# dacase/rnamotif

Hardware: AMD Instinct MI355X
Metric: Mbases scanned/sec (whole node) + hits/sec, trna.descr (higher is better)
Workload: dtype u8; 1 GPU; trna.descr (15 elements) over 100 x 1000000 base synthetic records per GPU (iid uniform acgt, numpy default_rng(20240601)), both strands; database resident in HBM (no upload in the step); bases_per_gpu=100000000, total_bases=100000000, candidates=5837, parallelism=1 GPU

## Files before the change

### rnamotif_amd/csrc/rm_efn2_core.h

```cpp
#pragma once
#include "rm_efn_core.h"

#define RME2_INF	RMA_EFN2_INFINITY
template< class Cand, int BIG = 0 >
struct rme2_ctx_t {
	static constexpr int	max_helix = BIG ? 52 : 16, stk = BIG ? 128 : 32;
	const rma_efn2data_t	*E;
	const Cand	*C;
	int	l_base;
	RMD_FN_MEMBER int	bc( int i ) const { return C->bc( i ); }
	RMD_FN_MEMBER int	bp( int i ) const { return C->bp( i ); }
};

RMD_FN int rme2_min( int a, int b ) { return a < b ? a : b; }

template< class X > RMD_FN int rme2_aupen( const X &x, int i, int j )
{
	return ( x.bc( i ) == RMA_BC_T || x.bc( j ) == RMA_BC_T ) ? x.E->auend : 0;
}
template< class X > RMD_FN int rme2_dangle( const X &x, int i, int j, int ip, int jp )
{
	return x.E->dangle[ x.bc( i ) ][ x.bc( j ) ][ x.bc( ip ) ][ jp ];
}
template< class X > RMD_FN int rme2_loginc( const X &x, int size )
// ... 101 lines not shown
	}
	if( closed )
		coax[ n ][ n ] = coax[ 0 ][ 0 ];
	const int	npair = closed ? n : n - 1;
	for( int h = 0; h < npair; h++ ){
		const int	d = hx[ h + 1 ][ 1 ] - hx[ h ][ 0 ];
		int	v = coax[ h ][ h ] + coax[ h + 1 ][ h + 1 ];
		if( d == 1 )
			v = rme2_min( v, RME2_T4( coax, hx[ h ][ 1 ], hx[ h ][ 0 ], hx[ h + 1 ][ 1 ], hx[ h + 1 ][ 0 ] ) );
		else if( d == 2 ){
			bool	g5, g3;
			if( closed ){
				g5 = h != 0 ? hx[ h ][ 1 ] - hx[ h - 1 ][ 0 ] > 1 : hx[ 0 ][ 1 ] - hx[ n - 1 ][ 0 ] > 1;
				g3 = h != n - 1 ? hx[ h + 2 ][ 1 ] - hx[ h + 1 ][ 0 ] > 1 : hx[ 1 ][ 1 ] - hx[ 0 ][ 0 ] > 1;
			}else{
				g5 = h != 0 ? hx[ h ][ 1 ] - hx[ h - 1 ][ 0 ] > 1 : hx[ 0 ][ 1 ] > 1;
				g3 = h != n - 2 ? hx[ h + 2 ][ 1 ] - hx[ h + 1 ][ 0 ] > 1 : hx[ n - 1 ][ 0 ] < l_base;
			}
			if( g5 ){
				const int	t = h != 0 ?
					RME2_T4( tstackcoax, hx[ h ][ 0 ], hx[ h ][ 1 ], hx[ h ][ 0 ] + 1, hx[ h ][ 1 ] - 1 ) :
					RME2_T4( tstackcoax, hx[ h ][ 1 ], hx[ h ][ 0 ], hx[ h ][ 0 ] + 1, hx[ h ][ 1 ] - 1 );
				v = rme2_min( v, t + RME2_T4( coaxstack, hx[ h ][ 0 ] + 1, hx[ h ][ 1 ] - 1, hx[ h + 1 ][ 1 ], hx[ h + 1 ][ 0 ] ) );
			}
			if( g3 )
				v = rme2_min( v, RME2_T4( tstackcoax, hx[ h ][ 0 ] + 1, hx[ h + 1 ][ 0 ] + 1, hx[ h + 1 ][ 1 ], hx[ h + 1 ][ 0 ] ) +
					RME2_T4( coaxstack, hx[ h ][ 0 ], hx[ h ][ 1 ], hx[ h ][ 0 ] + 1, hx[ h + 1 ][ 0 ] + 1 ) );
		}
		coax[ h ][ h + 1 ] = v;
	}
	for( int h = 2; h <= m && h < n; h++ )
		for( int a = 0; a + h <= m; a++ ){
			int	v = coax[ a ][ a ] + coax[ a + 1 ][ a + h ];
			for( int b = 1; b < h; b++ )
				v = rme2_min( v, coax[ a ][ a + b ] + coax[ a + b + 1 ][ a + h ] );
			coax[ a ][ a + h ] = v;
		}
	if( closed )
		return rme2_min( coax[ 0 ][ n - 1 ], coax[ 1 ][ n ] );
	return n >= 1 ? coax[ 0 ][ n - 1 ] : 0;
}

template< class X > RMD_FN int rme2_efn2( const X &x )
{
	const rma_efn2data_t	*e = x.E;
	const int	l_base = x.l_base;
	int	stk_i[ X::stk ], stk_j[ X::stk ], sp = 0;
	int	hx[ X::max_helix + 1 ][ 2 ];
	int	energy = 0;
	stk_i[ sp ] = 0;
	stk_j[ sp ] = l_base;
	sp++;
	while( sp > 0 ){
		sp--;
		int	i = stk_i[ sp ], j = stk_j[ sp ];
		if( i < 0 || j < 0 || i > l_base || j > l_base )
			return RME2_INF;
		if( x.bp( i ) == j ){
			if( i >= j )
				return RME2_INF;
			for( bool again = true; again; ){
				again = false;
				while( x.bp( i + 1 ) == j - 1 ){
					energy += RME2_T4( stack, i, j, i + 1, j - 1 ) + e->eparam[ 1 ];
					i++;
					j--;
				}
				int	n_helix = 0, ip = 0, jp = 0;
				for( int k = i + 1; k < j; ){
					const int	q = x.bp( k );
					if( q > k ){
						n_helix++;
						ip = k;
						k = q + 1;
						jp = q;
					}else if( q == -1 )
						k++;
					else
						return RME2_INF;
				}
				if( n_helix == 0 )
					energy += rme2_hploop( x, i, j );
				else if( n_helix == 1 ){
					energy += rme2_ibloop( x, i, j, ip, jp );
					i = ip;
					j = jp;
					again = true;
				}else{
					n_helix++;
					if( n_helix >= X::max_helix )
						return RME2_INF;
					hx[ 0 ][ 0 ] = i;
					hx[ 0 ][ 1 ] = j;
					int	n_upn = 0;
					for( int h = 1; h < n_helix; h++ ){
						int	p = hx[ h - 1 ][ 0 ] + 1;
						while( x.bp( p ) == -1 )
							p++;
						const int	q = x.bp( p );
						energy += rme2_aupen( x, p, q );
						hx[ h ][ 1 ] = p;
						hx[ h ][ 0 ] = q;
						if( sp >= X::stk )
							return RME2_INF;
						stk_i[ sp ] = p;
						stk_j[ sp ] = q;
						sp++;
						n_upn += p - hx[ h - 1 ][ 0 ] - 1;
					}
					hx[ n_helix ][ 0 ] = hx[ 0 ][ 0 ];
					hx[ n_helix ][ 1 ] = hx[ 0 ][ 1 ];
					n_upn += hx[ n_helix ][ 1 ] - hx[ n_helix - 1 ][ 0 ] - 1;
					energy += e->efn2a + n_helix * e->efn2c;
					energy += n_upn <= 6 ? n_upn * e->efn2b :
						6 * e->efn2b + e->mbl_log[ n_upn < RMA_EFN_LOGINC ? n_upn : RMA_EFN_LOGINC - 1 ];
					energy += rme2_branches( x, hx, n_helix, true );
				}
			}
			continue;
		}
		int	n_helix = 0;
		while( i < l_base ){
			const int	q = x.bp( i );
			if( q != -1 ){
				n_helix++;
				i = q;
			}
			i++;
		}
		if( n_helix >= X::max_helix )
			return RME2_INF;
		int	p = 1;
		for( int h = 0; h < n_helix; h++ ){
			while( p <= l_base && x.bp( p ) == 0 )
				p++;
			const int	q = p <= l_base ? x.bp( p ) : -1;
			if( q < 0 )
				return RME2_INF;
			energy += rme2_aupen( x, p, q );
			hx[ h ][ 1 ] = p;
			hx[ h ][ 0 ] = q;
			if( sp >= X::stk )
				return RME2_INF;
			stk_i[ sp ] = p;
			stk_j[ sp ] = q;
			sp++;
			p = q + 1;
		}
		energy += rme2_branches( x, hx, n_helix, false );
	}
	return energy;
}

template< class Seq, int BIG = 0 >
RMD_FN int rme2_site_energy( const rmd_program_t *P, const rma_efn2data_t *E, const Seq *sq, const int32_t *w, int k,
	int16_t *bpbuf = nullptr, uint8_t *bcbuf = nullptr, int cache = 0 )
{
	rme_cand_t<Seq>	c;
	c.P = P;
	c.w = w;
	c.sq = sq;
	if( !c.setup( rmd_efn_sites( P )[ k ] ) )
		return RME_INF;
	if( bpbuf != nullptr && c.len <= cache )
		c.fill_cache( bpbuf, bcbuf );
	rme2_ctx_t< rme_cand_t<Seq>, BIG >	x;
	x.E = E;
	x.C = &c;
	x.l_base = c.len - 1;
	return rme2_efn2( x );
}
```

### rnamotif_amd/csrc/rm_efn_core.h

```cpp
#pragma once
#include "rm_dev_program.h"

#ifndef RMD_FN
#define RMD_FN	static inline
#endif
#ifndef RMD_FN_MEMBER
#define RMD_FN_MEMBER	inline
#endif

enum {
	RME_INTER = 0,
	RME_BULGE = RME_INTER + 31,
	RME_HAIRPIN = RME_BULGE + 31,
	RME_DANGLE = RME_HAIRPIN + 31,
	RME_POPPEN = RME_DANGLE + 250,
	RME_EPARAM = RME_POPPEN + 5,
	RME_MISC = RME_EPARAM + 16,
	RME_TRIKEY = RME_MISC + 9,
	RME_TRIVAL = RME_TRIKEY + 50,
	RME_TLVAL = RME_TRIVAL + 50,
	RME_STACK = RME_TLVAL + 100,
	RME_TSTKH = RME_STACK + 625,
	RME_TSTKI = RME_TSTKH + 625,
	RME_SINT2 = RME_TSTKI + 625,
	RME_ASINT = RME_SINT2 + 900,
	RME_SINT4 = RME_ASINT + 4500,
	RME_N16 = RME_SINT4 + 22500
};
enum { RME_MAXPEN, RME_AUEND, RME_GUBONUS, RME_CSLOPE, RME_CINT, RME_C3, RME_GAIL, RME_NTRI, RME_NTL };

struct rme_tables_t {
	const int16_t	*t;
	const int32_t	*tlkey;
	const int32_t	*loginc;
};

template< class Cand, int BIG = 0 >
struct rme_ctx_t {
	static constexpr int	stk = BIG ? 128 : 48;
	const rme_tables_t	*T;
	const Cand	*C;
	int	l_base;
	RMD_FN_MEMBER int	bc( int i ) const { return C->bc( i ); }
	RMD_FN_MEMBER int	bp( int i ) const { return C->bp( i ); }
	RMD_FN_MEMBER int	tab( int off ) const { return T->t[ off ]; }
};

#define RME_INF	RMA_EFN_INFINITY

template< class X > RMD_FN int rme_dangle( const X &x, int i, int j, int ip, int jp )
{
	return x.tab( RME_DANGLE + ( ( x.bc( i ) * 5 + x.bc( j ) ) * 5 + x.bc( ip ) ) * 2 + jp );
}

template< class X > RMD_FN int rme_aupen( const X &x, int i, int j )
{
	int	bi = x.bc( i ), bj = x.bc( j );
	int	pen = ( bi == RMA_BC_A && bj == RMA_BC_T ) || ( bi == RMA_BC_G && bj == RMA_BC_T ) ||
		( bi == RMA_BC_T && ( bj == RMA_BC_A || bj == RMA_BC_G ) );
	return pen * x.tab( RME_MISC + RME_AUEND );
}

template< class X > RMD_FN int rme_tab4( const X &x, int base, int a, int b, int c, int d )
{
	return x.tab( base + ( ( a * 5 + b ) * 5 + c ) * 5 + d );
}

template< class X > RMD_FN int rme_loginc( const X &x, int size )
{
	return x.T->loginc[ size < RMA_EFN_LOGINC ? size : RMA_EFN_LOGINC - 1 ];
}

template< class X > RMD_FN int rme_stack( const X &x, int i, int j )
{
	if( i == x.l_base || j == x.l_base + 1 )
		return RME_INF;
	return rme_tab4( x, RME_STACK, x.bc( i ), x.bc( j ), x.bc( i + 1 ), x.bc( j - 1 ) ) + x.tab( RME_EPARAM + 0 );
}

RMD_FN int rme_wc( int i, int j ) { return i + j == 3; }
RMD_FN int rme_gu( int i, int j ) { return i == RMA_BC_G && j == RMA_BC_T; }

template< class X > RMD_FN int rme_ibloop( const X &x, int i, int j, int ip, int jp )
{
	if( ( i <= x.l_base && ip > x.l_base ) || ( jp <= x.l_base && j > x.l_base ) )
		return RME_INF;
	int	size1 = ip - i - 1, size2 = j - jp - 1, size = size1 + size2;
	int	m = size1 < size2 ? size1 : size2;
	int	min4 = m < 4 ? m : 4;
	int	si = x.bc( i ), sj = x.bc( j ), sip = x.bc( ip ), sjp = x.bc( jp );
	int	rval = 0;
	if( size1 == 0 || size2 == 0 ){
		if( size == 1 )
			return rme_tab4( x, RME_STACK, si, sj, sip, sjp ) + x.tab( RME_BULGE + size ) + x.tab( RME_EPARAM + 1 );
		rval = rme_aupen( x, i, j ) + rme_aupen( x, ip, jp );
		if( size > 30 )
			rval += x.tab( RME_BULGE + 30 ) + rme_loginc( x, size ) + x.tab( RME_EPARAM + 1 );
		else
			rval += x.tab( RME_BULGE + size ) + x.tab( RME_EPARAM + 1 );
		return rval;
	}
	int	lopsid = size1 > size2 ? size1 - size2 : size2 - size1;
	int	pen = lopsid * x.tab( RME_POPPEN + min4 );
	if( pen > x.tab( RME_MISC + RME_MAXPEN ) )
		pen = x.tab( RME_MISC + RME_MAXPEN );
	int	gail = ( size1 == 1 || size2 == 1 ) && x.tab( RME_MISC + RME_GAIL ) == 1;
	if( size > 30 ){
		if( gail )
			rval += rme_tab4( x, RME_TSTKI, si, sj, RMA_BC_A, RMA_BC_A ) + rme_tab4( x, RME_TSTKI, sjp, sip, RMA_BC_A, RMA_BC_A );
		else
			rval += rme_tab4( x, RME_TSTKI, si, sj, x.bc( i + 1 ), x.bc( j - 1 ) ) +
				rme_tab4( x, RME_TSTKI, sjp, sip, x.bc( jp + 1 ), x.bc( ip - 1 ) );
		rval += x.tab( RME_INTER + 30 ) + rme_loginc( x, size ) + x.tab( RME_EPARAM + 2 ) + pen;
	}else if( lopsid == 1 && size == 3 ){
		int	lf, rt;
		if( size1 < size2 ){
			if( rme_wc( si, sj ) ) lf = si;
			else if( rme_gu( si, sj ) ) lf = 4;
			else if( rme_gu( sj, si ) ) lf = 5;
			else return RME_INF;
			if( rme_wc( sip, sjp ) ) rt = sip;
			else if( rme_gu( sip, sjp ) ) rt = 4;
			else if( rme_gu( sjp, sip ) ) rt = 5;
			else return RME_INF;
			rval += x.tab( RME_EPARAM + 2 ) + x.tab( RME_ASINT + ( ( ( lf * 6 + rt ) * 5 + x.bc( i + 1 ) ) * 5 + x.bc( j - 1 ) ) * 5 + x.bc( jp + 1 ) );
		}else{
			if( rme_wc( sjp, sip ) ) lf = sjp;
			else if( rme_gu( sjp, sip ) ) lf = 4;
			else if( rme_gu( sip, sjp ) ) lf = 5;
			else return RME_INF;
			if( rme_wc( sj, si ) ) rt = sj;
			else if( rme_gu( sj, si ) ) rt = 4;
			else if( rme_gu( si, sj ) ) rt = 5;
			else return RME_INF;
			rval += x.tab( RME_EPARAM + 2 ) + x.tab( RME_ASINT + ( ( ( lf * 6 + rt ) * 5 + x.bc( jp + 1 ) ) * 5 + x.bc( ip - 1 ) ) * 5 + x.bc( i + 1 ) );
		}
	}else if( lopsid == 0 && size <= 4 ){
		int	lf, rt;
		if( rme_wc( si, sj ) ) lf = si;
		else if( rme_gu( si, sj ) || rme_gu( sj, si ) ) lf = si + 2;
		else return RME_INF;
		if( rme_wc( sip, sjp ) ) rt = sip;
		else if( rme_gu( sip, sjp ) || rme_gu( sjp, sip ) ) rt = sip + 2;
		else return RME_INF;
		if( size == 2 )
			rval += x.tab( RME_EPARAM + 2 ) + x.tab( RME_SINT2 + ( ( lf * 6 + rt ) * 5 + x.bc( i + 1 ) ) * 5 + x.bc( j - 1 ) );
		else if( size == 4 )
			rval += x.tab( RME_EPARAM + 2 ) + x.tab( RME_SINT4 + ( ( ( ( lf * 6 + rt ) * 5 + x.bc( i + 1 ) ) * 5 + x.bc( j - 1 ) ) * 5 + x.bc( ip - 1 ) ) * 5 + x.bc( jp + 1 ) );
	}else{
		if( gail )
			rval += rme_tab4( x, RME_TSTKI, si, sj, RMA_BC_A, RMA_BC_A ) + rme_tab4( x, RME_TSTKI, sjp, sip, RMA_BC_A, RMA_BC_A );
		else
			rval += rme_tab4( x, RME_TSTKI, si, sj, x.bc( i + 1 ), x.bc( j - 1 ) ) +
				rme_tab4( x, RME_TSTKI, sjp, sip, x.bc( jp + 1 ), x.bc( ip - 1 ) );
// ... 65 lines not shown
	int	sp = 0, e = 0;
	stk_i[ 0 ] = 0;
	stk_j[ 0 ] = x.l_base;
	stk_open[ 0 ] = 1;
	sp = 1;
	const int	fbp = x.tab( RME_EPARAM + 5 ), helixp = x.tab( RME_EPARAM + 8 );
	while( sp > 0 ){
		sp--;
		int	i = stk_i[ sp ], j = stk_j[ sp ];
		int	open = int( ( stk_open[ sp >> 6 ] >> ( sp & 63 ) ) & 1 );
		int	fb = open ? 0 : fbp;
		int	done = 0;
		const int	e_call = e;
		if( x.bp( i ) == -1 || x.bp( j ) == -1 ){
			while( x.bp( i ) == -1 && x.bp( i + 1 ) == -1 ){
				i++;
				e += fb;
				if( i >= j - 1 ){
					done = 1;
					break;
				}
			}
			if( done )
				continue;
			while( x.bp( j ) == -1 && x.bp( j - 1 ) == -1 ){
				j--;
				e += fb;
				if( i >= j - 1 ){
					done = 1;
					break;
				}
			}
			if( done )
				continue;
			if( x.bp( i ) == -1 && x.bp( i + 1 ) > i + 1 ){
				int	dg = rme_dangle( x, x.bp( i + 1 ), i + 1, i, 1 );
				e += ( dg < 0 ? dg : 0 ) + fb;
				i++;
			}
			if( x.bp( j ) == -1 && x.bp( j - 1 ) != -1 && x.bp( j - 1 ) < j - 1 ){
				int	dg = rme_dangle( x, j - 1, x.bp( j - 1 ), j, 0 );
				e += ( dg < 0 ? dg : 0 ) + fb;
				j--;
			}
		}
		if( x.bp( i ) != j ){
			int	k = x.bp( i ), kp = x.bp( j );
			if( k >= kp || sp + 2 > RME_STK ){
				e = e_call + RME_INF;
				continue;
			}
			int	cut;
			if( x.bp( k + 1 ) != -1 )
				cut = k;
			else if( x.bp( k + 2 ) == -1 )
				cut = k + 1;
			else if( rme_dangle( x, k, i, k + 1, 0 ) <= rme_dangle( x, x.bp( k + 2 ), k + 2, k + 1, 1 ) )
				cut = k + 1;
			else
				cut = k;
			stk_i[ sp ] = cut + 1;
			stk_j[ sp ] = j;
			stk_open[ sp >> 6 ] = ( stk_open[ sp >> 6 ] & ~( 1ull << ( sp & 63 ) ) ) | ( ( unsigned long long )open << ( sp & 63 ) );
			sp++;
			stk_i[ sp ] = i;
			stk_j[ sp ] = cut;
			stk_open[ sp >> 6 ] = ( stk_open[ sp >> 6 ] & ~( 1ull << ( sp & 63 ) ) ) | ( ( unsigned long long )open << ( sp & 63 ) );
			sp++;
			continue;
		}
		if( !open )
			e += helixp;
		e += rme_aupen( x, i, j );
		for( ; ; ){
			if( x.bp( i + 1 ) == j - 1 ){
				e += rme_stack( x, i, j );
				i++;
				j--;
				continue;
			}
			int	sum = 0, ip = 0, jp = 0, bad = 0;
			for( int k = i + 1; k < j; ){
				int	b = x.bp( k );
				if( b > k ){
					sum++;
					ip = k;
					k = b + 1;
					jp = k - 1;
					if( k > j ){
						bad = 1;
						break;
					}
				}else if( b == -1 )
					k++;
				else{
					bad = 1;
					break;
				}
			}
			if( bad ){
				e = e_call + RME_INF;
				break;
			}
			if( sum == 0 ){
				e += rme_hploop( x, i, j );
				break;
			}
			if( sum == 1 ){
				e += rme_ibloop( x, i, j, ip, jp );
				i = ip;
				j = jp;
				continue;
			}
			int	is = i + 1, js = j - 1;
			e += x.tab( RME_EPARAM + 4 ) + helixp + rme_aupen( x, i, j );
			if( x.bp( i + 1 ) == -1 && x.bp( i + 2 ) != -1 ){
				int	dg = rme_dangle( x, i, j, i + 1, 0 );
				if( dg <= rme_dangle( x, x.bp( i + 2 ), i + 2, i + 1, 1 ) ){
					is = i + 2;
					e += ( dg < 0 ? dg : 0 ) + fbp;
				}
			}
			if( x.bp( i + 1 ) == -1 && x.bp( i + 2 ) == -1 ){
				int	dg = rme_dangle( x, i, j, i + 1, 0 );
				is = i + 2;
				e += ( dg < 0 ? dg : 0 ) + fbp;
			}
			if( x.bp( j - 1 ) == -1 && x.bp( j - 2 ) != -1 ){
				int	dg = rme_dangle( x, i, j, j - 1, 1 );
				if( dg <= rme_dangle( x, j - 2, x.bp( j - 2 ), j - 1, 0 ) ){
					js = j - 2;
					e += ( dg < 0 ? dg : 0 ) + fbp;
				}
			}
			if( x.bp( j - 1 ) == -1 && x.bp( j - 2 ) == -1 ){
				int	dg = rme_dangle( x, i, j, j - 1, 1 );
				js = j - 2;
				e += ( dg < 0 ? dg : 0 ) + fbp;
			}
			if( sp + 1 > RME_STK ){
				e += RME_INF;
				break;
			}
			stk_i[ sp ] = is;
			stk_j[ sp ] = js;
			stk_open[ sp >> 6 ] &= ~( 1ull << ( sp & 63 ) );
			sp++;
			break;
		}
	}
	return e;
}

template< class Seq >
struct rme_cand_t {
	const rmd_program_t	*P;
	const int32_t	*w;
	const Seq	*sq;
	int	idx, idx2, pos, pos2;
	int	off5, start, len;
	int16_t	*cbp = nullptr;
	uint8_t	*cbc = nullptr;

	RMD_FN_MEMBER int	moff( int d ) const { return w[ RMA_HIT_HDR + 4 * d ]; }
	RMD_FN_MEMBER int	mlen( int d ) const { return w[ RMA_HIT_HDR + 4 * d + 1 ]; }

	RMD_FN_MEMBER int	setup( const rma_efn_site_t &es )
	{
		idx = es.idx;
		idx2 = es.idx2;
		pos = es.pos;
		pos2 = es.pos2 < 0 ? mlen( idx2 ) - 1 : es.pos2;
		off5 = moff( idx );
		start = off5 + pos;
		len = 0;
		for( int d = idx; d <= idx2; d++ ){
			int	t = P->elems[ d ].type;
			if( t != RMA_T_SS && t != RMA_T_H5 && t != RMA_T_H3 )
				return 0;
			len += mlen( d );
		}
		len -= pos;
		len -= mlen( idx2 ) - ( pos2 + 1 );
		if( len <= 0 )
			return 0;
		for( int d = idx; d <= idx2; d++ ){
			const rmd_elem_t	&st = P->elems[ d ];
			if( st.type == RMA_T_SS || ( st.type == RMA_T_H5 && d == idx2 ) || ( st.type == RMA_T_H3 && d == idx ) )
				continue;
			if( !st.proper )
				return 0;
			int	m = st.mates[ 0 ];
			int	p0 = d == idx ? pos : 0, p1 = d == idx2 ? pos2 + 1 : mlen( d );
			if( p0 >= p1 )
				continue;
			int	lo = ( mlen( m ) - ( p1 - 1 ) - 1 ) + moff( m ) - off5;
			int	hi = ( mlen( m ) - p0 - 1 ) + moff( m ) - off5;
			if( lo < 0 || hi >= len )
				return 0;
		}
		return 1;
	}
	RMD_FN_MEMBER void	fill_cache( int16_t *bpbuf, uint8_t *bcbuf )
	{
		for( int d = idx; d <= idx2; d++ ){
			const rmd_elem_t	&st = P->elems[ d ];
			const int	p0 = d == idx ? pos : 0, p1 = d == idx2 ? pos2 + 1 : mlen( d );
			const bool	ss = st.type == RMA_T_SS || ( st.type == RMA_T_H5 && d == idx2 ) || ( st.type == RMA_T_H3 && d == idx );
			const int	m = st.mates[ 0 ];
			const int	ps = P->efn_usestdbp ? P->efn_stdbp : st.pairset;
			for( int pq = p0; pq < p1; pq++ ){
				const int	p = moff( d ) + pq, i = p - start;
				const int	b = sq->code( p );
				bcbuf[ i ] = uint8_t( b );
				int	partner = -1;
				if( !ss ){
					const int	q1 = mlen( m ) - pq - 1;
					const int	b1 = sq->code( q1 + moff( m ) );
					if( ( rmd_pairsets( P )[ ps ].mat2 >> ( b * 5 + b1 ) ) & 1 )
						partner = q1 + moff( m ) - off5;
				}
				bpbuf[ i ] = int16_t( partner );
			}
		}
		cbp = bpbuf;
		cbc = bcbuf;
	}
	RMD_FN_MEMBER int	bc( int i ) const
	{
		if( i < 0 || i >= len )
			return RMA_BC_N;
		if( cbc != nullptr )
			return cbc[ i ];
		return sq->code( start + i );
	}
	RMD_FN_MEMBER int	bp( int i ) const
	{
		if( i < 0 || i >= len )
			return -1;
		if( cbp != nullptr )
			return cbp[ i ];
		int	p = start + i;
		for( int d = idx; d <= idx2; d++ ){
			int	o = moff( d ), l = mlen( d );
			if( p < o || p >= o + l )
				continue;
			const rmd_elem_t	&st = P->elems[ d ];
			if( st.type == RMA_T_SS || ( st.type == RMA_T_H5 && d == idx2 ) || ( st.type == RMA_T_H3 && d == idx ) )
				return -1;
			int	pq = p - o;
			int	m = st.mates[ 0 ];
			int	q1 = mlen( m ) - pq - 1;
			int	ps = P->efn_usestdbp ? P->efn_stdbp : st.pairset;
			int	b = sq->code( p ), b1 = sq->code( q1 + moff( m ) );
			return ( ( rmd_pairsets( P )[ ps ].mat2 >> ( b * 5 + b1 ) ) & 1 ) ? q1 + moff( m ) - off5 : -1;
		}
		return -1;
	}
};

template< class Seq, int BIG = 0 >
RMD_FN int rme_site_energy( const rmd_program_t *P, const rme_tables_t *T, const Seq *sq, const int32_t *w, int k,
	int16_t *bpbuf = nullptr, uint8_t *bcbuf = nullptr, int cache = 0 )
{
	rme_cand_t<Seq>	c;
	c.P = P;
	c.w = w;
	c.sq = sq;
	if( !c.setup( rmd_efn_sites( P )[ k ] ) )
		return RME_INF;
	if( bpbuf != nullptr && c.len <= cache )
		c.fill_cache( bpbuf, bcbuf );
	rme_ctx_t< rme_cand_t<Seq>, BIG >	x;
	x.T = T;
	x.C = &c;
	x.l_base = c.len - 1;
	return rme_efn( x );
}
```

### rnamotif_amd/csrc/rm_scan_kernel.h

```cpp
#pragma once
#include <hip/hip_runtime.h>
#include <cstdint>

#define RMD_HD		__host__ __device__ inline
#define RMD_FN		static __device__ inline
#define RMD_COLD	static __device__ inline
#define RMD_FN_MEMBER	__device__ inline
#include "rm_scan_core.h"
#include "rm_efn_core.h"
#include "rm_efn2_core.h"
#include "rm_kernels.h"

__device__ inline int db_code( const DbView &db, int64_t base )
{
	uint32_t	am = db.amask[ base >> 5 ];
	if( ( am >> ( base & 31 ) ) & 1 )
		return RMA_BC_N;
	return ( db.codes[ base >> 4 ] >> ( 2 * ( base & 15 ) ) ) & 3;
}

__device__ inline int db_strand_code( const DbView &db, int64_t off, int slen, int comp, int p )
{
	int	c = db_code( db, off + ( comp ? slen - 1 - p : p ) );
	return ( comp && c < 4 ) ? 3 - c : c;
// ... 1948 lines not shown
								int	whole;
								k = pool_item_begin<BLOCK>( P, db, pool + RMK_POOL_WORDS * size_t( i ), col, NIB_MAX, lr, st, nsq, sink.seq, sink.comp, whole );
							}else
								dry = true;
						}
						if( ( dbg & RMK_DBG_CYCLES ) && lane_id == 0 )
							atomicAdd( rmk_ctr<RMK_C_POP_CYCLES>( hb ), __builtin_amdgcn_s_memtime() - t_p0 );
						continue;
					}
					if( busy == 0 )
						break;
					const unsigned long long	t_s0 = ( dbg & RMK_DBG_CYCLES ) ? __builtin_amdgcn_s_memtime() : 0;
					if( ( dbg & RMK_DBG_CYCLES ) && lane_id == 0 ){
						atomicAdd( rmk_ctr<RMK_C_STEPS>( hb ), 1ull );
						atomicAdd( rmk_ctr<RMK_C_STEP_LANES>( hb ), ( unsigned long long )__popcll( busy ) );
					}
					int	k_in_ = 0;
					if( dbg & RMK_DBG_CYCLES ){
						k_in_ = k;
						for( int o = 32; o > 0; o >>= 1 )
							k_in_ = rmd_imax( k_in_, __shfl_xor( k_in_, o ) );
					}
					if( k >= 0 )
						k = rmd_lean_step<LdsRecs<BLOCK>, DevSink, rmd_nibseq_t<BLOCK>, rmd_no_accel_t, true>( P, lr, st, nsq, k, &lane, sink, none );
					const unsigned long long	t_e0 = ( dbg & RMK_DBG_CYCLES ) ? __builtin_amdgcn_s_memtime() : 0;
					const int	n_em_ = ( dbg & RMK_DBG_CYCLES ) ? __popcll( __ballot( k >= 0 && st.pending ) ) : 0;
					wave_emit_pending<BLOCK>( P, lr, st, k, [ & ]( int l ){
						return rmd_nibseq_t<BLOCK>{ nsq.w + ( l - lane_id ), __shfl( nsq.flip, l ), __shfl( nsq.bias, l ) }; },
						sink.seq, sink.comp, hb, lane_id );
					if( ( dbg & RMK_DBG_CYCLES ) && lane_id == 0 && n_em_ ){
						atomicAdd( rmk_ctr<RMK_C_EMIT_CYCLES>( hb ), __builtin_amdgcn_s_memtime() - t_e0 );
						atomicAdd( rmk_ctr<RMK_C_EMITTED>( hb ), ( unsigned long long )n_em_ );
					}
					if( ( dbg & RMK_DBG_CYCLES ) && lane_id == 0 ){
						const unsigned long long	dt_ = __builtin_amdgcn_s_memtime() - t_s0;
						atomicAdd( rmk_ctr<RMK_C_STEP_CYCLES>( hb ), dt_ );
						atomicMax( rmk_ctr<RMK_C_STEP_LONGEST>( hb ), dt_ );
						atomicAdd( rmk_ctr<RMK_C_STEP_LOG2>( hb ) + ( 63 - __clzll( dt_ | 1ull ) ), 1ull );
						atomicAdd( rmk_ctr<RMK_C_LEVEL_CYCLES>( hb ) + rmd_imin( rmd_imax( k_in_, 0 ), 15 ), dt_ );
						atomicAdd( rmk_ctr<RMK_C_LEVEL_STEPS>( hb ) + rmd_imin( rmd_imax( k_in_, 0 ), 15 ), 1ull );
						t_wave += dt_;
						atomicMax( rmk_ctr<RMK_C_WAVE_MOST>( hb ), t_wave );
					}
				}
				__syncthreads();
				if( tid == 0 ){
					s_pool_n = 0;
					s_pool_head = 0;
				}
			}
			if( last ){
				PHASE( 4 );
				if( ( dbg & RMK_DBG_TIMELINE ) && tid == 0 && had_tiles ){
					atomicMax( rmk_ctr<RMK_C_TL_DONE_MAX>( hb ), ( unsigned long long )wall_clock64() );
					atomicAdd( rmk_ctr<RMK_C_TL_DONE_SUM>( hb ), ( unsigned long long )wall_clock64() );
				}
				break;
			}
			}
		}else if constexpr( LEAN ){

			rmd_lean_t	st;
			TailAccel	accel{ P, pb, tile, pb_words, p_lo, vec_words * 64, tail_from_rows ? 0 : -1 };
			for( ; ; ){
				unsigned long long	t_b0 = ( dbg & RMK_DBG_CYCLES ) ? __builtin_amdgcn_s_memtime() : 0;
				for( unsigned long long want; ( want = __ballot( k < 0 && !dry ) ) != 0; ){
					if( ( dbg & RMK_DBG_CYCLES ) && lane_id == 0 ){
						atomicAdd( rmk_ctr<RMK_C_POP_ROUNDS>( hb ), 1ull );
						atomicAdd( rmk_ctr<RMK_C_POP_LANES>( hb ), ( unsigned long long )__popcll( want ) );
					}
					int	base = 0;
					if( lane_id == __ffsll( want ) - 1 )
						base = atomicAdd( &s_qhead, __popcll( want ) );
					base = __shfl( base, __ffsll( want ) - 1 );
					if( k < 0 && !dry ){
						const int	i = base + __popcll( want & lt_mask );
						if( i < nq ){
							const unsigned	item = i < qcap ? queue[ i ] :
								__hip_atomic_load( spill + ( i - qcap ), __ATOMIC_RELAXED, __HIP_MEMORY_SCOPE_AGENT );
							const int	r = int( item & 0xffffu );
							if constexpr( G > 1 ){
								const int	sl = int( item >> 26 );
								const int	*c = s_ctx[ sl ];
								slen = c[ 2 ];
								z0 = c[ 3 ];
								p_lo = c[ 4 ];
								tile = tile0 + size_t( sl ) * slot_bytes;
								pb = pb0 + ( size_t( sl ) * n_vec + 1 ) * pb_words;
								sq = rmd_seq_t{ tile, p_lo };
								sink.seq = c[ 0 ];
								sink.comp = c[ 1 ];
								accel.pb = pb;
								accel.tile = tile;
								accel.p_lo = p_lo;
								accel.vec_bits = c[ 5 ] * 64;
							}
							const int	szero = z0 + int( ( item >> 16 ) & ( G > 1 ? 0x3ffu : 0xffffu ) );
							bool	drop = false;
							if( accel.usable_for >= 0 && r != 0xffff ){
								int	hi, lo;
								rmd_level0_range( P, szero, slen, &hi, &lo );
								const int	span = hi - r - szero + 1;
								drop = true;
								for( int hl = e0.minlen; hl <= e0.maxlen && drop; hl++ ){
									const int	ilen = span - 2 * hl;
									if( ilen < e0.minilen )
										break;
									bool	ok;
									if( ilen <= e0.maxilen && ( !accel.tail( e0, szero, hl, span - 1 - hl, &ok ) || ok ) )
										drop = false;
								}
							}
							if( !drop )
								k = rmd_lean_begin( P, lr, st, szero, slen,
									r == 0xffff ? 0 : r, r == 0xffff ? RMD_ALL_RANKS : 1 );
						}else
							dry = true;
					}
				}
				const unsigned long long	busy = __ballot( k >= 0 );
				unsigned long long	t_b1 = 0;
				if( dbg & RMK_DBG_CYCLES ){
					t_b1 = __builtin_amdgcn_s_memtime();
					if( lane_id == 0 ){
						atomicAdd( rmk_ctr<RMK_C_POP_CYCLES>( hb ), t_b1 - t_b0 );
						atomicAdd( rmk_ctr<RMK_C_STEPS>( hb ), 1ull );
						atomicAdd( rmk_ctr<RMK_C_STEP_LANES>( hb ), ( unsigned long long )__popcll( busy ) );
					}
				}
				if( busy == 0 )
					break;
				if( k >= 0 )
					k = rmd_lean_step<LdsRecs<BLOCK>, DevSink, rmd_seq_t, TailAccel, true>( P, lr, st, sq, k, &lane, sink, accel );
				wave_emit_pending<BLOCK>( P, lr, st, k, [ & ]( int l ){
					return rmd_seq_t{ tile0 + __shfl( int( sq.sq - tile0 ), l ), __shfl( sq.sq0, l ) }; },
					sink.seq, sink.comp, hb, lane_id );
				if( ( dbg & RMK_DBG_CYCLES ) && lane_id == 0 )
					atomicAdd( rmk_ctr<RMK_C_STEP_CYCLES>( hb ), __builtin_amdgcn_s_memtime() - t_b1 );
			}
		}else{
			GenTile	gt{ P, lean_lo, g_before, g_deep, queue, spill, qcap, nq, &s_qhead, &s_dqn, &s_dqhead,
				pb, tile, pb_words, p_lo, vec_words, slen, z0, split_s, dbg,
				ConcatCtx{ db.base_off, db.slen, CONCAT ? db.concat_bases : 0ll, seq, ent_n } };
			general_pass_b<BLOCK, KINDS, CONCAT>( gt, sink );
		}
		PHASE( 4 );
		__syncthreads();
		PHASE( 5 );
	}
#undef PHASE
}

struct DevSeq {
	DbView	db;
	int64_t	off;
	int	slen, comp;
	__device__ inline int code( int p ) const { return db_strand_code( db, off, slen, comp, p ); }
};

#define RME_N16_PAD	( ( RME_N16 + 7 ) / 8 * 8 )
#define EFN_CACHE	96
#define EFN_LIGHT_LDS	( 64 * ( ( EFN_CACHE + 2 ) * 2 + EFN_CACHE + 4 ) )
template< int BLOCK, int BIG, bool STAGE >
__device__ __forceinline__ void efn_body( const rmd_program_t *gP, const DbView &db, int32_t *hits, long long n_hits,
	const int16_t *g16, const int32_t *tlkey, const int32_t *loginc, const rma_efn2data_t *e2 )
{
	__shared__ __align__( 16 ) int16_t	t16_s[ STAGE ? RME_N16_PAD : 8 ];
	const int16_t	*t16 = g16;
	if constexpr( STAGE ){
		if( g16 != nullptr )
			for( int i = threadIdx.x; i < RME_N16_PAD / 8; i += BLOCK )
				reinterpret_cast<uint4 *>( t16_s )[ i ] = reinterpret_cast<const uint4 *>( g16 )[ i ];
		__syncthreads();
		t16 = t16_s;
	}
	__shared__ int16_t	s_bp[ STAGE ? BLOCK : 1 ][ EFN_CACHE + 1 ];
	__shared__ uint8_t	s_bc[ STAGE ? BLOCK : 1 ][ EFN_CACHE + 4 ];
	rme_tables_t	T{ t16, tlkey, loginc };
	int16_t	*bpbuf = s_bp[ STAGE ? threadIdx.x : 0 ];
	uint8_t	*bcbuf = s_bc[ STAGE ? threadIdx.x : 0 ];
	if constexpr( !STAGE ){
		extern __shared__ __align__( 16 ) unsigned char	efn_dyn[];
		bpbuf = reinterpret_cast<int16_t *>( efn_dyn ) + threadIdx.x * ( EFN_CACHE + 2 );
		bcbuf = efn_dyn + BLOCK * ( EFN_CACHE + 2 ) * sizeof( int16_t ) + threadIdx.x * ( EFN_CACHE + 4 );
	}
	const int	efn_off = RMA_HIT_HDR + 4 * gP->n_elems + 4;
	for( long long h = ( long long )blockIdx.x * BLOCK + threadIdx.x; h < n_hits; h += ( long long )gridDim.x * BLOCK ){
		int32_t	*w = hits + h * gP->hit_stride;
		DevSeq	sq{ db, db.base_off[ w[ 0 ] ], db.slen[ w[ 0 ] ], w[ 1 ] };
		for( int k = 0; k < gP->n_efn; k++ ){
			if( rmd_efn_sites( gP )[ k ].kind == RMA_EFN_KIND_EFN2 )
				w[ efn_off + k ] = e2 != nullptr ? rme2_site_energy<DevSeq, BIG>( gP, e2, &sq, w, k, bpbuf, bcbuf, EFN_CACHE ) : RME2_INF;
			else if( g16 != nullptr )
				w[ efn_off + k ] = rme_site_energy<DevSeq, BIG>( gP, &T, &sq, w, k, bpbuf, bcbuf, EFN_CACHE );
		}
	}
}

template< int BLOCK, int BIG = 0 >
__global__ void __launch_bounds__( BLOCK )
rma_efn_kernel( const rmd_program_t *gP, DbView db, int32_t *hits, long long n_hits,
	const int16_t *g16, const int32_t *tlkey, const int32_t *loginc, const rma_efn2data_t *e2 )
{
	efn_body<BLOCK, BIG, true>( gP, db, hits, n_hits, g16, tlkey, loginc, e2 );
}

template< int BIG = 0 >
__global__ void __launch_bounds__( 64, 4 )
rma_efn_light_kernel( const rmd_program_t *gP, DbView db, int32_t *hits, long long n_hits,
	const int16_t *g16, const int32_t *tlkey, const int32_t *loginc, const rma_efn2data_t *e2 )
{
	__builtin_amdgcn_s_setprio( 3 );
	efn_body<64, BIG, false>( gP, db, hits, n_hits, g16, tlkey, loginc, e2 );
}

#define RMK_DEFINE_LAUNCHER( name_, LEAN_, G_, KINDS_, POOL_, ... ) \
hipError_t name_( int grid, size_t lds, hipStream_t s, const rmk_search_args &a ) \
{ \
	constexpr int	BLOCK_ = ( LEAN_ ) ? SEARCH_BLOCK : GENERAL_BLOCK; \
	auto	kernel = &rma_search_kernel<BLOCK_, LEAN_, G_, KINDS_, POOL_ __VA_OPT__(,) __VA_ARGS__>; \
	hipError_t	e = hipFuncSetAttribute( reinterpret_cast<const void *>( kernel ), hipFuncAttributeMaxDynamicSharedMemorySize, int( lds ) ); \
	if( e != hipSuccess ) \
		return e; \
	 \
	{ \
		static thread_local size_t	for_lds = ~size_t( 0 ); \
		static thread_local int	resident = 0, for_dev = -1; \
		int	dev = 0; \
		( void )hipGetDevice( &dev ); \
		if( for_lds != lds || for_dev != dev ){ \
			int	per_cu = 0, cus = 0; \
			resident = 0; \
			if( hipOccupancyMaxActiveBlocksPerMultiprocessor( &per_cu, kernel, BLOCK_, lds ) == hipSuccess && \
				hipDeviceGetAttribute( &cus, hipDeviceAttributeMultiprocessorCount, dev ) == hipSuccess ) \
				resident = per_cu * cus; \
			for_lds = lds; \
			for_dev = dev; \
		} \
		if( resident > 0 && grid > resident ) \
			grid = resident; \
	} \
	hipLaunchKernelGGL( kernel, dim3( grid ), dim3( BLOCK_ ), lds, s, \
		a.d_prog, a.prog_bytes, a.qcap, a.db, a.hb, a.tile_bytes, a.dbg ); \
	return hipGetLastError(); \
}

#define RMK_DEFINE_DRAIN_LAUNCHER( name_ ) \
hipError_t name_( int grid, size_t lds, hipStream_t s, const rmk_search_args &a ) \
{ \
	auto	kernel = &rma_drain_kernel<DRAIN_BLOCK>; \
	hipError_t	e = hipFuncSetAttribute( reinterpret_cast<const void *>( kernel ), hipFuncAttributeMaxDynamicSharedMemorySize, int( lds ) ); \
	if( e != hipSuccess ) \
		return e; \
	hipLaunchKernelGGL( kernel, dim3( grid ), dim3( DRAIN_BLOCK ), lds, s, a.d_prog, a.prog_bytes, a.db, a.hb, a.tile_bytes, a.dbg ); \
	return hipGetLastError(); \
}
```

Baseline: 165,900 Mbases/s.

## Decode EFN candidate base windows in bulk and stage element facts in LDS

The EFN cache fill now decodes a candidate's whole base window from a few packed code and ambiguity-mask words at once, instead of one strided global read per base. Partner bases are looked up in that local window. Per-element type, mate and pair-matrix facts are precomputed once per block into shared memory, so each candidate no longer walks the program struct and pairset table. Pointers are also marked restrict. The trade-offs are more register use for the unrolled word arrays and a block-wide sync at kernel start.

```diff
diff --git a/profiles/efn_window.py b/profiles/efn_window.py
--- /dev/null
+++ b/profiles/efn_window.py
@@ -0,0 +1,53 @@
+import json
+import os
+import statistics
+import sys
+import time
+
+ROOT = os.path.dirname(os.path.dirname(os.path.abspath(__file__)))
+sys.path.insert(0, ROOT)
+import rnamotif_amd as R
+
+tag, out = sys.argv[1], sys.argv[2]
+os.environ.setdefault("EFNDATA", R.EFNDATA_DIR)
+d = R.Descriptor(["-descr", os.path.join(ROOT, "tests", "golden", "descr", "trna.descr")])
+seqs = R.synthetic_records(100)
+scs = [R.Scanner(d), R.Scanner(d)]
+db = scs[0].database(seqs)
+for s in scs:
+    s.attach(db)
+
+
+def turns(n):
+    pend = None
+    for i in range(n):
+        s = scs[i & 1]
+        s.scan_begin(db)
+        if pend is not None:
+            pend.scan_end(copy=False)
+        pend = s
+    return pend.scan_end(copy=False).shape[0]
+
+
+row = {"lib": tag}
+for light in (1, 0):
+    scs[0].set_option("efn_light", light)
+    for rep in range(3):
+        scs[0].scan_device(db)
+    ks = []
+    for rep in range(12):
+        scs[0].scan_device(db)
+        ks.append(round(scs[0].last_kernel_ms()[2], 4))
+    row["efn_light_ms" if light else "efn_staged_ms"] = {"median": statistics.median(ks), "min": min(ks), "max": max(ks), "all": ks}
+scs[0].set_option("efn_light", -1)
+turns(20)
+ms = []
+for rep in range(5):
+    t0 = time.perf_counter()
+    cand = turns(200)
+    ms.append(round((time.perf_counter() - t0) / 200 * 1e3, 4))
+row["ms_per_step_in_turns"] = ms
+row["candidates"] = cand
+print(json.dumps(row), flush=True)
+with open(out, "a") as f:
+    f.write(json.dumps(row) + "\n")
diff --git a/rnamotif_amd/csrc/rm_efn2_core.h b/rnamotif_amd/csrc/rm_efn2_core.h
--- a/rnamotif_amd/csrc/rm_efn2_core.h
+++ b/rnamotif_amd/csrc/rm_efn2_core.h
@@ -277,19 +277,20 @@
 	return energy;
 }
 
-template< class Seq, int BIG = 0 >
+template< class Seq, int BIG = 0, bool FACTS = false >
 RMD_FN int rme2_site_energy( const rmd_program_t *P, const rma_efn2data_t *E, const Seq *sq, const int32_t *w, int k,
-	int16_t *bpbuf = nullptr, uint8_t *bcbuf = nullptr, int cache = 0 )
-{
-	rme_cand_t<Seq>	c;
+	int16_t *bpbuf = nullptr, uint8_t *bcbuf = nullptr, int cache = 0, const rme_el_t *el = nullptr )
+{
+	rme_cand_t<Seq, FACTS>	c;
 	c.P = P;
 	c.w = w;
 	c.sq = sq;
+	c.F = el;
 	if( !c.setup( rmd_efn_sites( P )[ k ] ) )
 		return RME_INF;
 	if( bpbuf != nullptr && c.len <= cache )
 		c.fill_cache( bpbuf, bcbuf );
-	rme2_ctx_t< rme_cand_t<Seq>, BIG >	x;
+	rme2_ctx_t< rme_cand_t<Seq, FACTS>, BIG >	x;
 	x.E = E;
 	x.C = &c;
 	x.l_base = c.len - 1;
diff --git a/rnamotif_amd/csrc/rm_efn_core.h b/rnamotif_amd/csrc/rm_efn_core.h
--- a/rnamotif_amd/csrc/rm_efn_core.h
+++ b/rnamotif_amd/csrc/rm_efn_core.h
@@ -1,5 +1,8 @@
 #pragma once
+#include <type_traits>
+#include <utility>
 #include "rm_dev_program.h"
+#include "rm_seq_window.h"
 
 #ifndef RMD_FN
 #define RMD_FN	static inline
@@ -371,11 +374,39 @@
 	return e;
 }
 
-template< class Seq >
+template< class Seq, class = void > struct rme_has_window : std::false_type {};
+template< class Seq > struct rme_has_window< Seq,
+	std::void_t< decltype( std::declval<const Seq &>().window( 0, 0, static_cast<uint8_t *>( nullptr ) ) ) > > : std::true_type {};
+
+struct rme_el_t {
+	uint32_t	mat2;
+	int8_t	type, proper, mate, pad;
+};
+RMD_FN rme_el_t rme_el_of( const rmd_program_t *P, int d )
+{
+	const rmd_elem_t	&st = P->elems[ d ];
+	rme_el_t	e{ 0, st.type, st.proper, st.mates[ 0 ], 0 };
+	if( st.type == RMA_T_H5 || st.type == RMA_T_H3 ){
+		const int	ps = P->efn_usestdbp ? P->efn_stdbp : st.pairset;
+		if( ps >= 0 )
+			e.mat2 = rmd_pairsets( P )[ ps ].mat2;
+	}
+	return e;
+}
+
+template< class Seq, bool FACTS = false >
 struct rme_cand_t {
 	const rmd_program_t	*P;
 	const int32_t	*w;
 	const Seq	*sq;
+	const rme_el_t	*F = nullptr;
+	RMD_FN_MEMBER rme_el_t	el( int d ) const
+	{
+		if constexpr( FACTS )
+			return F[ d ];
+		else
+			return rme_el_of( P, d );
+	}
 	int	idx, idx2, pos, pos2;
 	int	off5, start, len;
 	int16_t	*cbp = nullptr;
@@ -394,7 +425,7 @@
 		start = off5 + pos;
 		len = 0;
 		for( int d = idx; d <= idx2; d++ ){
-			int	t = P->elems[ d ].type;
+			int	t = el( d ).type;
 			if( t != RMA_T_SS && t != RMA_T_H5 && t != RMA_T_H3 )
 				return 0;
 			len += mlen( d );
@@ -404,12 +435,12 @@
 		if( len <= 0 )
 			return 0;
 		for( int d = idx; d <= idx2; d++ ){
-			const rmd_elem_t	&st = P->elems[ d ];
+			const rme_el_t	st = el( d );
 			if( st.type == RMA_T_SS || ( st.type == RMA_T_H5 && d == idx2 ) || ( st.type == RMA_T_H3 && d == idx ) )
 				continue;
 			if( !st.proper )
 				return 0;
-			int	m = st.mates[ 0 ];
+			int	m = st.mate;
 			int	p0 = d == idx ? pos : 0, p1 = d == idx2 ? pos2 + 1 : mlen( d );
 			if( p0 >= p1 )
 				continue;
@@ -422,24 +453,29 @@
 	}
 	RMD_FN_MEMBER void	fill_cache( int16_t *bpbuf, uint8_t *bcbuf )
 	{
+		if constexpr( rme_has_window<Seq>::value )
+			sq->window( start, len, bcbuf );
+		else
+			for( int i = 0; i < len; i++ )
+				bcbuf[ i ] = uint8_t( sq->code( start + i ) );
 		for( int d = idx; d <= idx2; d++ ){
-			const rmd_elem_t	&st = P->elems[ d ];
+			const rme_el_t	st = el( d );
+			const int	od = moff( d ) - start;
 			const int	p0 = d == idx ? pos : 0, p1 = d == idx2 ? pos2 + 1 : mlen( d );
 			const bool	ss = st.type == RMA_T_SS || ( st.type == RMA_T_H5 && d == idx2 ) || ( st.type == RMA_T_H3 && d == idx );
-			const int	m = st.mates[ 0 ];
-			const int	ps = P->efn_usestdbp ? P->efn_stdbp : st.pairset;
+			if( ss ){
+				for( int pq = p0; pq < p1; pq++ )
+					bpbuf[ od + pq ] = -1;
+				continue;
+			}
+			const int	m = st.mate;
+			const uint32_t	mat2 = st.mat2;
+			const int	qm = mlen( m ) - 1 + moff( m );
 			for( int pq = p0; pq < p1; pq++ ){
-				const int	p = moff( d ) + pq, i = p - start;
-				const int	b = sq->code( p );
-				bcbuf[ i ] = uint8_t( b );
-				int	partner = -1;
-				if( !ss ){
-					const int	q1 = mlen( m ) - pq - 1;
-					const int	b1 = sq->code( q1 + moff( m ) );
-					if( ( rmd_pairsets( P )[ ps ].mat2 >> ( b * 5 + b1 ) ) & 1 )
-						partner = q1 + moff( m ) - off5;
-				}
-				bpbuf[ i ] = int16_t( partner );
+				const int	b = bcbuf[ od + pq ];
+				const int	j = qm - pq - start;
+				const int	b1 = j >= 0 && j < len ? bcbuf[ j ] : sq->code( qm - pq );
+				bpbuf[ od + pq ] = int16_t( ( ( mat2 >> ( b * 5 + b1 ) ) & 1 ) ? qm - pq - off5 : -1 );
 			}
 		}
 		cbp = bpbuf;
@@ -464,33 +500,33 @@
 			int	o = moff( d ), l = mlen( d );
 			if( p < o || p >= o + l )
 				continue;
-			const rmd_elem_t	&st = P->elems[ d ];
+			const rme_el_t	st = el( d );
 			if( st.type == RMA_T_SS || ( st.type == RMA_T_H5 && d == idx2 ) || ( st.type == RMA_T_H3 && d == idx ) )
 				return -1;
 			int	pq = p - o;
-			int	m = st.mates[ 0 ];
+			int	m = st.mate;
 			int	q1 = mlen( m ) - pq - 1;
-			int	ps = P->efn_usestdbp ? P->efn_stdbp : st.pairset;
 			int	b = sq->code( p ), b1 = sq->code( q1 + moff( m ) );
-			return ( ( rmd_pairsets( P )[ ps ].mat2 >> ( b * 5 + b1 ) ) & 1 ) ? q1 + moff( m ) - off5 : -1;
+			return ( ( st.mat2 >> ( b * 5 + b1 ) ) & 1 ) ? q1 + moff( m ) - off5 : -1;
 		}
 		return -1;
 	}
 };
 
-template< class Seq, int BIG = 0 >
+template< class Seq, int BIG = 0, bool FACTS = false >
 RMD_FN int rme_site_energy( const rmd_program_t *P, const rme_tables_t *T, const Seq *sq, const int32_t *w, int k,
-	int16_t *bpbuf = nullptr, uint8_t *bcbuf = nullptr, int cache = 0 )
-{
-	rme_cand_t<Seq>	c;
+	int16_t *bpbuf = nullptr, uint8_t *bcbuf = nullptr, int cache = 0, const rme_el_t *el = nullptr )
+{
+	rme_cand_t<Seq, FACTS>	c;
 	c.P = P;
 	c.w = w;
 	c.sq = sq;
+	c.F = el;
 	if( !c.setup( rmd_efn_sites( P )[ k ] ) )
 		return RME_INF;
 	if( bpbuf != nullptr && c.len <= cache )
 		c.fill_cache( bpbuf, bcbuf );
-	rme_ctx_t< rme_cand_t<Seq>, BIG >	x;
+	rme_ctx_t< rme_cand_t<Seq, FACTS>, BIG >	x;
 	x.T = T;
 	x.C = &c;
 	x.l_base = c.len - 1;
diff --git a/rnamotif_amd/csrc/rm_scan_kernel.h b/rnamotif_amd/csrc/rm_scan_kernel.h
--- a/rnamotif_amd/csrc/rm_scan_kernel.h
+++ b/rnamotif_amd/csrc/rm_scan_kernel.h
@@ -2124,18 +2124,27 @@
 }
 
 struct DevSeq {
-	DbView	db;
+	const uint32_t	*codes, *amask;
 	int64_t	off;
 	int	slen, comp;
-	__device__ inline int code( int p ) const { return db_strand_code( db, off, slen, comp, p ); }
+	__device__ inline int code( int p ) const
+	{
+		const int64_t	base = off + ( comp ? slen - 1 - p : p );
+		if( ( amask[ base >> 5 ] >> ( base & 31 ) ) & 1 )
+			return RMA_BC_N;
+		const int	c = ( codes[ base >> 4 ] >> ( 2 * ( base & 15 ) ) ) & 3;
+		return comp ? 3 - c : c;
+	}
+	__device__ inline void window( int p, int n, uint8_t *out ) const { rmw_window_codes( codes, amask, off, slen, comp, p, n, out ); }
 };
 
 #define RME_N16_PAD	( ( RME_N16 + 7 ) / 8 * 8 )
 #define EFN_CACHE	96
+static_assert( EFN_CACHE <= RMW_MAX, "a cached call is one window of DevSeq::window()" );
 #define EFN_LIGHT_LDS	( 64 * ( ( EFN_CACHE + 2 ) * 2 + EFN_CACHE + 4 ) )
 template< int BLOCK, int BIG, bool STAGE >
-__device__ __forceinline__ void efn_body( const rmd_program_t *gP, const DbView &db, int32_t *hits, long long n_hits,
-	const int16_t *g16, const int32_t *tlkey, const int32_t *loginc, const rma_efn2data_t *e2 )
+__device__ __forceinline__ void efn_body( const rmd_program_t * __restrict__ gP, const DbView &db, int32_t * __restrict__ hits, long long n_hits,
+	const int16_t * __restrict__ g16, const int32_t * __restrict__ tlkey, const int32_t * __restrict__ loginc, const rma_efn2data_t * __restrict__ e2 )
 {
 	__shared__ __align__( 16 ) int16_t	t16_s[ STAGE ? RME_N16_PAD : 8 ];
 	const int16_t	*t16 = g16;
@@ -2156,31 +2165,35 @@
 		bpbuf = reinterpret_cast<int16_t *>( efn_dyn ) + threadIdx.x * ( EFN_CACHE + 2 );
 		bcbuf = efn_dyn + BLOCK * ( EFN_CACHE + 2 ) * sizeof( int16_t ) + threadIdx.x * ( EFN_CACHE + 4 );
 	}
+	__shared__ rme_el_t	s_el[ RMD_MAX_ELEMS ];
+	for( int d = threadIdx.x; d < gP->n_elems; d += BLOCK )
+		s_el[ d ] = rme_el_of( gP, d );
+	__syncthreads();
 	const int	efn_off = RMA_HIT_HDR + 4 * gP->n_elems + 4;
 	for( long long h = ( long long )blockIdx.x * BLOCK + threadIdx.x; h < n_hits; h += ( long long )gridDim.x * BLOCK ){
 		int32_t	*w = hits + h * gP->hit_stride;
-		DevSeq	sq{ db, db.base_off[ w[ 0 ] ], db.slen[ w[ 0 ] ], w[ 1 ] };
+		DevSeq	sq{ db.codes, db.amask, db.base_off[ w[ 0 ] ], db.slen[ w[ 0 ] ], w[ 1 ] };
 		for( int k = 0; k < gP->n_efn; k++ ){
 			if( rmd_efn_sites( gP )[ k ].kind == RMA_EFN_KIND_EFN2 )
-				w[ efn_off + k ] = e2 != nullptr ? rme2_site_energy<DevSeq, BIG>( gP, e2, &sq, w, k, bpbuf, bcbuf, EFN_CACHE ) : RME2_INF;
+				w[ efn_off + k ] = e2 != nullptr ? rme2_site_energy<DevSeq, BIG, true>( gP, e2, &sq, w, k, bpbuf, bcbuf, EFN_CACHE, s_el ) : RME2_INF;
 			else if( g16 != nullptr )
-				w[ efn_off + k ] = rme_site_energy<DevSeq, BIG>( gP, &T, &sq, w, k, bpbuf, bcbuf, EFN_CACHE );
+				w[ efn_off + k ] = rme_site_energy<DevSeq, BIG, true>( gP, &T, &sq, w, k, bpbuf, bcbuf, EFN_CACHE, s_el );
 		}
 	}
 }
 
 template< int BLOCK, int BIG = 0 >
 __global__ void __launch_bounds__( BLOCK )
-rma_efn_kernel( const rmd_program_t *gP, DbView db, int32_t *hits, long long n_hits,
-	const int16_t *g16, const int32_t *tlkey, const int32_t *loginc, const rma_efn2data_t *e2 )
+rma_efn_kernel( const rmd_program_t * __restrict__ gP, DbView db, int32_t * __restrict__ hits, long long n_hits,
+	const int16_t * __restrict__ g16, const int32_t * __restrict__ tlkey, const int32_t * __restrict__ loginc, const rma_efn2data_t * __restrict__ e2 )
 {
 	efn_body<BLOCK, BIG, true>( gP, db, hits, n_hits, g16, tlkey, loginc, e2 );
 }
 
 template< int BIG = 0 >
 __global__ void __launch_bounds__( 64, 4 )
-rma_efn_light_kernel( const rmd_program_t *gP, DbView db, int32_t *hits, long long n_hits,
-	const int16_t *g16, const int32_t *tlkey, const int32_t *loginc, const rma_efn2data_t *e2 )
+rma_efn_light_kernel( const rmd_program_t * __restrict__ gP, DbView db, int32_t * __restrict__ hits, long long n_hits,
+	const int16_t * __restrict__ g16, const int32_t * __restrict__ tlkey, const int32_t * __restrict__ loginc, const rma_efn2data_t * __restrict__ e2 )
 {
 	__builtin_amdgcn_s_setprio( 3 );
 	efn_body<64, BIG, false>( gP, db, hits, n_hits, g16, tlkey, loginc, e2 );
diff --git a/rnamotif_amd/csrc/rm_seq_window.h b/rnamotif_amd/csrc/rm_seq_window.h
--- /dev/null
+++ b/rnamotif_amd/csrc/rm_seq_window.h
@@ -0,0 +1,49 @@
+#pragma once
+#include <stdint.h>
+#include "rm_dev_program.h"
+
+#ifndef RMD_FN
+#define RMD_FN	static inline
+#endif
+
+#define RMW_MAX		96
+#define RMW_AWORDS	( ( 31 + RMW_MAX + 31 ) / 32 )
+#define RMW_CWORDS	( ( 15 + RMW_MAX + 15 ) / 16 )
+
+RMD_FN void rmw_window_codes( const uint32_t *codes, const uint32_t *amask, int64_t off, int slen, int comp, int p, int n, uint8_t *out )
+{
+	const int64_t	f0 = off + ( comp ? slen - p - n : p ), f1 = f0 + n - 1;
+	const int64_t	a0 = f0 >> 5, c0 = f0 >> 4;
+	const int	na = int( ( f1 >> 5 ) - a0 ), nc = int( ( f1 >> 4 ) - c0 );
+	uint32_t	am[ RMW_AWORDS ], cw[ RMW_CWORDS ];
+#pragma unroll
+	for( int k = 0; k < RMW_AWORDS; k++ )
+		am[ k ] = amask[ a0 + ( k < na ? k : na ) ];
+#pragma unroll
+	for( int k = 0; k < RMW_CWORDS; k++ )
+		cw[ k ] = codes[ c0 + ( k < nc ? k : nc ) ];
+	const int	odd = int( c0 & 1 );
+#pragma unroll
+	for( int k = 0; k < RMW_CWORDS; k++ ){
+		if( k > nc )
+			break;
+		const uint32_t	w = cw[ k ];
+		static_assert( RMW_CWORDS >> 1 < RMW_AWORDS, "an odd first codes word" );
+		const uint32_t	mw = odd ? am[ ( k + 1 ) >> 1 ] : am[ k >> 1 ];
+		const uint32_t	m = ( ( odd + k ) & 1 ) ? mw >> 16 : mw & 0xffffu;
+		const int64_t	b0 = ( c0 + k ) << 4;
+		const int	lo = k == 0 ? int( f0 - b0 ) : 0, hi = k == nc ? int( f1 - b0 ) : 15;
+#ifdef __clang__
+#pragma clang loop vectorize( disable ) unroll( disable )
+#endif
+		for( int r = lo; r <= hi; r++ ){
+			const int	j = int( b0 - f0 ) + r;
+			int	c = ( w >> ( 2 * r ) ) & 3;
+			if( comp )
+				c = 3 - c;
+			if( ( m >> r ) & 1 )
+				c = RMA_BC_N;
+			out[ comp ? n - 1 - j : j ] = uint8_t( c );
+		}
+	}
+}
```

Result: faster. 174,300 Mbases/s, median of 6 (+5.1%).
